# giuliojiang/pbrt-v3-IILE

Measured on AMD Instinct MI355X. Metric: Mray/s on killeroo-simple 1080p (path integrator, rays = Scene::Intersect + IntersectP calls), higher is better.
Workload: dtype f32

## Files before the change

pbrt-v3-iile_amd/csrc/device/dbsdf.h:

```cpp
#pragma once
enum Lobe : int { kLobePassThrough, kLobeLambert, kLobeLambertTrans, kLobeMicro, kLobeMicroTrans, kLobeBlend, kLobeSpecular, kLobeSpecTrans };
DEV bool lobe_is_specular(Lobe l) { return l == kLobePassThrough || l == kLobeSpecular || l == kLobeSpecTrans; }
struct Bsdf {
    F3 ns, ng, ss, ts;
    F3 kd;
    union { F3 micro_r, ks; };
    union { F3 kr, ltrans_t, cond_eta; };
    union { F3 kt, mtrans_t, cond_k; };
    float alpha, eta;
    float alpha_y;
    F3 t0;
    bool has_t0, has_t1;
    float path_eta;
    bool has_mtrans;
    int n_lobes;
    float on_a, on_b;
    bool oren_nayar;
    int mtype;
    bool has_lambert, has_micro, has_spec;
    bool has_blend;
    bool has_ltrans;
};
DEV int n_nonspec(const Bsdf &b) {
    return (b.has_lambert ? 1 : 0) + (b.has_ltrans ? 1 : 0) + (b.has_micro ? 1 : 0) + (b.has_mtrans ? 1 : 0) + (b.has_blend ? 1 : 0);
// ... 214 lines not shown
    *slope_y = Sg * z * sqrtf(1.f + *slope_x * *slope_x);
}
DEV F3 tr_sample_wh(F3 wo, float u0, float u1, float ax, float ay) {
    bool flip = wo.z < 0;
    F3 wi = flip ? -wo : wo;
    F3 ws = normalize(F3{ax * wi.x, ay * wi.y, wi.z});
    float sx, sy;
    tr_sample11(ws.z, u0, u1, &sx, &sy);
    float tmp = cos_phi(ws) * sx - sin_phi(ws) * sy;
    sy = sin_phi(ws) * sx + cos_phi(ws) * sy;
    sx = tmp;
    sx = ax * sx;
    sy = ay * sy;
    F3 wh = normalize(F3{-sx, -sy, 1.f});
    if (flip) wh = -wh;
    return wh;
}
DEV F3 micro_f(const Bsdf &b, F3 wo, F3 wi) {
    float cos_o = fabsf(wo.z), cos_i = fabsf(wi.z);
    F3 wh = wi + wo;
    if (cos_i == 0 || cos_o == 0) return F3{0, 0, 0};
    if (wh.x == 0 && wh.y == 0 && wh.z == 0) return F3{0, 0, 0};
    wh = normalize(wh);
    F3 F;
    if (b.mtype == kMatMetal) {
        F = fr_conductor(fabsf(dot(wi, wh)), b.cond_eta, b.cond_k);
    } else {
        float Fr = (b.mtype == kMatUber || b.mtype == kMatGlass || b.mtype == kMatTranslucent) ? fr_dielectric(dot(wi, wh), 1.f, b.eta)
                                                                                              : fr_dielectric(dot(wi, wh), 1.5f, 1.f);
        F = F3{Fr, Fr, Fr};
    }
    return sdiv(b.micro_r * tr_d(wh, b.alpha, b.alpha_y) * tr_g(wo, wi, b.alpha, b.alpha_y) * F, 4 * cos_i * cos_o);
}
DEV float micro_pdf(const Bsdf &b, F3 wo, F3 wi) {
    if (!same_hemisphere(wo, wi)) return 0;
    F3 wh = normalize(wo + wi);
    return tr_pdf(wo, wh, b.alpha, b.alpha_y) / (4 * dot(wo, wh));
}
DEV float pow5(float v) { return (v * v) * (v * v) * v; }
DEV F3 blend_f(const Bsdf &b, F3 wo, F3 wi) {
    const F3 one = F3{1.f, 1.f, 1.f};
    const F3 diffuse = (28.f / (23.f * kPi)) * b.kd * (one - b.ks) * (1 - pow5(1 - .5f * fabsf(wi.z))) * (1 - pow5(1 - .5f * fabsf(wo.z)));
    F3 wh = wi + wo;
    if (wh.x == 0 && wh.y == 0 && wh.z == 0) return F3{0, 0, 0};
    wh = normalize(wh);
    const float s = tr_d(wh, b.alpha, b.alpha_y) / (4 * absdot(wi, wh) * mx(fabsf(wi.z), fabsf(wo.z)));
    const F3 schlick = b.ks + pow5(1 - dot(wi, wh)) * (one - b.ks);
    return diffuse + s * schlick;
}
DEV float blend_pdf(const Bsdf &b, F3 wo, F3 wi) {
    if (!same_hemisphere(wo, wi)) return 0;
    const F3 wh = normalize(wo + wi);
    const float pdf_wh = tr_pdf(wo, wh, b.alpha, b.alpha_y);
    return .5f * (fabsf(wi.z) * kInvPi + pdf_wh / (4 * dot(wo, wh)));
}
DEV F3 diffuse_f(const Bsdf &b, F3 wo, F3 wi) {
    if (!b.oren_nayar) return b.kd * kInvPi;
    const float sin_i = sin_theta(wi), sin_o = sin_theta(wo);
    float max_cos = 0;
    if (double(sin_i) > 1e-4 && double(sin_o) > 1e-4) {
        const float sin_phi_i = sin_phi(wi), cos_phi_i = cos_phi(wi);
        const float sin_phi_o = sin_phi(wo), cos_phi_o = cos_phi(wo);
        const float d_cos = cos_phi_i * cos_phi_o + sin_phi_i * sin_phi_o;
        max_cos = mx(0.f, d_cos);
    }
    float sin_alpha, tan_beta;
    if (fabsf(wi.z) > fabsf(wo.z)) {
        sin_alpha = sin_o;
        tan_beta = sin_i / fabsf(wi.z);
    } else {
        sin_alpha = sin_i;
        tan_beta = sin_o / fabsf(wo.z);
    }
    return b.kd * kInvPi * (b.on_a + b.on_b * max_cos * sin_alpha * tan_beta);
}
DEV float lambert_pdf(F3 wo, F3 wi) { return same_hemisphere(wo, wi) ? fabsf(wi.z) * kInvPi : 0; }
DEV F3 ltrans_f(const Bsdf &b) { return b.ltrans_t * kInvPi; }
DEV float ltrans_pdf(F3 wo, F3 wi) { return !same_hemisphere(wo, wi) ? fabsf(wi.z) * kInvPi : 0; }
DEV bool refract_dir(F3 wi, F3 n, float eta, F3 *wt) {
    const float cos_i = dot(n, wi);
    const float sin2_i = mx(0.f, 1 - cos_i * cos_i);
    const float sin2_t = eta * eta * sin2_i;
    if (sin2_t >= 1) return false;
    const float cos_t = sqrtf(1 - sin2_t);
    *wt = eta * -wi + (eta * cos_i - cos_t) * n;
    return true;
}
DEV bool specular_refract(F3 wo, float eta_a, float eta_b, F3 *wi, float *scale) {
    const bool entering = wo.z > 0;
    const float eta_i = entering ? eta_a : eta_b, eta_t = entering ? eta_b : eta_a;
    const F3 n = (wo.z < 0.f) ? -F3{0, 0, 1} : F3{0, 0, 1};
    if (!refract_dir(wo, n, eta_i / eta_t, wi)) return false;
    *scale = (eta_i * eta_i) / (eta_t * eta_t);
    return true;
}
DEV F3 mtrans_f(const Bsdf &b, F3 wo, F3 wi) {
    if (same_hemisphere(wo, wi)) return F3{0, 0, 0};
    const float cos_o = wo.z, cos_i = wi.z;
    if (cos_i == 0 || cos_o == 0) return F3{0, 0, 0};
    const float eta_a = 1.f, eta_b = b.eta;
    const float eta = wo.z > 0 ? (eta_b / eta_a) : (eta_a / eta_b);
    F3 wh = normalize(wo + wi * eta);
    if (wh.z < 0) wh = -wh;
    const float F = fr_dielectric(dot(wo, wh), eta_a, eta_b);
    const float sqrt_denom = dot(wo, wh) + eta * dot(wi, wh);
    const float factor = 1 / eta;
    const float omf = 1.f - F;
    return F3{omf, omf, omf} * b.mtrans_t *
           fabsf(tr_d(wh, b.alpha, b.alpha_y) * tr_g(wo, wi, b.alpha, b.alpha_y) * eta * eta * absdot(wi, wh) * absdot(wo, wh) * factor * factor /
                 (cos_i * cos_o * sqrt_denom * sqrt_denom));
}
DEV float mtrans_pdf(const Bsdf &b, F3 wo, F3 wi) {
    if (same_hemisphere(wo, wi)) return 0;
    const float eta_a = 1.f, eta_b = b.eta;
    const float eta = wo.z > 0 ? (eta_b / eta_a) : (eta_a / eta_b);
    const F3 wh = normalize(wo + wi * eta);
    const float sqrt_denom = dot(wo, wh) + eta * dot(wi, wh);
    const float dwh_dwi = fabsf((eta * eta * dot(wi, wh)) / (sqrt_denom * sqrt_denom));
    return tr_pdf(wo, wh, b.alpha, b.alpha_y) * dwh_dwi;
}
DEV F3 lobes_f(const Bsdf &b, F3 wo, F3 wi) {
    F3 f = F3{0, 0, 0};
    if (b.has_lambert) f = f + diffuse_f(b, wo, wi);
    if (b.has_micro) f = f + micro_f(b, wo, wi);
    if (b.has_blend) f = f + blend_f(b, wo, wi);
    return f;
}
DEV F3 trans_lobes_f(const Bsdf &b, F3 wo, F3 wi) {
    F3 f = F3{0, 0, 0};
    if (b.has_ltrans) f = f + ltrans_f(b);
    if (b.has_mtrans) f = f + mtrans_f(b, wo, wi);
    return f;
}
DEV F3 bsdf_f(const Bsdf &b, F3 woW, F3 wiW) {
    F3 wi = to_local(b, wiW), wo = to_local(b, woW);
    if (wo.z == 0) return F3{0, 0, 0};
    bool reflect = dot(wiW, b.ng) * dot(woW, b.ng) > 0;
    if (reflect) return lobes_f(b, wo, wi);
    return trans_lobes_f(b, wo, wi);
}
DEV float bsdf_pdf(const Bsdf &b, F3 woW, F3 wiW) {
    if (b.n_lobes == 0) return 0.f;
    F3 wo = to_local(b, woW), wi = to_local(b, wiW);
    if (wo.z == 0) return 0.f;
    float pdf = 0.f;
    if (b.has_lambert) pdf += lambert_pdf(wo, wi);
    if (b.has_ltrans) pdf += ltrans_pdf(wo, wi);
    if (b.has_micro) pdf += micro_pdf(b, wo, wi);
    if (b.has_mtrans) pdf += mtrans_pdf(b, wo, wi);
    if (b.has_blend) pdf += blend_pdf(b, wo, wi);
    const int matching = n_nonspec(b);
    return matching > 0 ? pdf / matching : 0.f;
}
DEV F3 bsdf_sample_f(const Bsdf &b, F3 woW, F3 *wiW, float u0, float u1, float *pdf, const bool allow_specular = false,
                     bool *sampled_specular = nullptr, bool *sampled_transmission = nullptr) {
    if (sampled_specular) *sampled_specular = false;
    if (sampled_transmission) *sampled_transmission = false;
    const int matching = allow_specular ? b.n_lobes : n_nonspec(b);
    if (matching == 0) {
        *pdf = 0;
        return F3{0, 0, 0};
    }
    int comp = int(floorf(u0 * matching));
    if (comp > matching - 1) comp = matching - 1;
    Lobe pick;
    int count = comp;
    if (allow_specular && b.has_t0 && count-- == 0)
        pick = kLobePassThrough;
    else if (b.has_lambert && count-- == 0)
        pick = kLobeLambert;
    else if (b.has_ltrans && count-- == 0)
        pick = kLobeLambertTrans;
    else if (b.has_micro && count-- == 0)
        pick = kLobeMicro;
    else if (b.has_mtrans && count-- == 0)
        pick = kLobeMicroTrans;
    else if (b.has_blend && count-- == 0)
        pick = kLobeBlend;
    else if (!(allow_specular && b.has_t1) || (b.has_spec && count-- == 0))
        pick = kLobeSpecular;
    else
        pick = kLobeSpecTrans;
    if (pick == kLobeSpecular && !b.has_spec) __builtin_unreachable();
    const float ur0 = mn(u0 * matching - comp, kOneMinusEpsilon);
    F3 wo = to_local(b, woW);
    if (wo.z == 0) return F3{0, 0, 0};
    *pdf = 0;
    F3 wi = F3{0, 0, 0}, f;
    if (pick == kLobeLambert) {
        wi = cosine_sample_hemisphere(ur0, u1);
        if (wo.z < 0) wi.z *= -1;
        *pdf = lambert_pdf(wo, wi);
        f = diffuse_f(b, wo, wi);
    } else if (pick == kLobeLambertTrans) {
        wi = cosine_sample_hemisphere(ur0, u1);
        if (wo.z > 0) wi.z *= -1;
        *pdf = ltrans_pdf(wo, wi);
        f = ltrans_f(b);
    } else if (pick == kLobeMicro) {
        F3 wh = tr_sample_wh(wo, ur0, u1, b.alpha, b.alpha_y);
        wi = -wo + 2 * dot(wo, wh) * wh;
        if (!same_hemisphere(wo, wi))
            f = F3{0, 0, 0};
        else {
            *pdf = tr_pdf(wo, wh, b.alpha, b.alpha_y) / (4 * dot(wo, wh));
            f = micro_f(b, wo, wi);
        }
    } else if (pick == kLobeBlend) {
        float ua = ur0;
        if (ua < .5f) {
            ua = mn(2 * ua, kOneMinusEpsilon);
            wi = cosine_sample_hemisphere(ua, u1);
            if (wo.z < 0) wi.z *= -1;
        } else {
            ua = mn(2 * (ua - .5f), kOneMinusEpsilon);
            const F3 wh = tr_sample_wh(wo, ua, u1, b.alpha, b.alpha_y);
            wi = -wo + 2 * dot(wo, wh) * wh;
            if (!same_hemisphere(wo, wi)) return F3{0, 0, 0};
        }
        *pdf = blend_pdf(b, wo, wi);
        f = blend_f(b, wo, wi);
    } else if (pick == kLobeMicroTrans) {
        const F3 wh = tr_sample_wh(wo, ur0, u1, b.alpha, b.alpha_y);
        const float eta_a = 1.f, eta_b = b.eta;
        const float eta = wo.z > 0 ? (eta_a / eta_b) : (eta_b / eta_a);
        if (!refract_dir(wo, wh, eta, &wi)) return F3{0, 0, 0};
        *pdf = mtrans_pdf(b, wo, wi);
        f = mtrans_f(b, wo, wi);
    } else if (pick == kLobePassThrough || pick == kLobeSpecTrans) {
        const float eta_a = 1.f, eta_b = pick == kLobePassThrough ? 1.f : b.eta;
        float scale;
        if (!specular_refract(wo, eta_a, eta_b, &wi, &scale)) return F3{0, 0, 0};
        *pdf = 1;
        const F3 ft = (pick == kLobePassThrough ? b.t0 : b.kt) * (1.f - fr_dielectric(wi.z, eta_a, eta_b));
        f = sdiv(ft * scale, fabsf(wi.z));
        if (sampled_specular) *sampled_specular = true;
        if (sampled_transmission) *sampled_transmission = true;
    } else if (b.mtype == kMatGlass) {
        const float eta_a = 1.f, eta_b = b.eta;
        const float F = fr_dielectric(wo.z, eta_a, eta_b);
        if (ur0 < F) {
            wi = F3{-wo.x, -wo.y, wo.z};
            *pdf = F;
            f = sdiv(F * b.kr, fabsf(wi.z));
        } else {
            float scale;
            if (!specular_refract(wo, eta_a, eta_b, &wi, &scale)) return F3{0, 0, 0};
            const F3 ft = b.kt * (1 - F);
            *pdf = 1 - F;
            f = sdiv(ft * scale, fabsf(wi.z));
            if (sampled_transmission) *sampled_transmission = true;
        }
        if (sampled_specular) *sampled_specular = true;
    } else {
        wi = F3{-wo.x, -wo.y, wo.z};
        *pdf = 1;
        const float fr = b.mtype == kMatMirror ? 1.f : fr_dielectric(wi.z, 1.f, b.eta);
        f = sdiv(F3{fr, fr, fr} * b.kr, fabsf(wi.z));
        if (sampled_specular) *sampled_specular = true;
    }
    if (*pdf == 0) {
        if (sampled_specular) *sampled_specular = false;
        if (sampled_transmission) *sampled_transmission = false;
        return F3{0, 0, 0};
    }
    *wiW = to_world(b, wi);
    const bool glossy = !lobe_is_specular(pick);
    if (glossy && matching > 1) {
        if (pick != kLobeLambert && b.has_lambert) *pdf += lambert_pdf(wo, wi);
        if (pick != kLobeLambertTrans && b.has_ltrans) *pdf += ltrans_pdf(wo, wi);
        if (pick != kLobeMicro && b.has_micro) *pdf += micro_pdf(b, wo, wi);
        if (pick != kLobeMicroTrans && b.has_mtrans) *pdf += mtrans_pdf(b, wo, wi);
    }
    if (matching > 1) *pdf /= matching;
    if (glossy && matching > 1) {
        bool reflect = dot(*wiW, b.ng) * dot(woW, b.ng) > 0;
        f = reflect ? lobes_f(b, wo, wi) : trans_lobes_f(b, wo, wi);
    }
    return f;
}

enum DisneyLobe : int { kDzDiffuse, kDzFakeSS, kDzRetro, kDzSheen, kDzMicro, kDzCoat, kDzMicroTrans, kDzLambertTrans };
struct DisneyBsdf : Bsdf {
    bool disney;
    bool dz_diffuse;
    bool dz_thin, dz_sheen, dz_coat;
    bool dz_trans_smith;
    F3 r_diffuse, r_ss, r_retro, r_sheen;
    F3 cspec0;
    float metallic, rough;
    float coat_w, coat_alpha;
    float t_ax, t_ay;
};
template <bool DIS>
struct bsdf_of { using type = Bsdf; };
template <>
struct bsdf_of<true> { using type = DisneyBsdf; };
DEV float lerpf(float t, float a, float b) { return (1 - t) * a + t * b; }
DEV F3 lerp3(float t, F3 a, F3 b) { return (1 - t) * a + t * b; }
DEV float sqr(float x) { return x * x; }
DEV float schlick_weight(float cos_theta) {
    const float m = clampf(1 - cos_theta, 0, 1);
    return (m * m) * (m * m) * m;
}
DEV float fr_schlick(float r0, float cos_theta) { return lerpf(schlick_weight(cos_theta), r0, 1.f); }
DEV F3 fr_schlick3(F3 r0, float cos_theta) { return lerp3(schlick_weight(cos_theta), r0, F3{1.f, 1.f, 1.f}); }
DEV float schlick_r0_from_eta(float eta) { return sqr(eta - 1) / sqr(eta + 1); }

DEV void make_disney(const DMaterial &m, const iile_disney &dz, DisneyBsdf *b) {
    b->disney = true;
    b->mtype = kMatDisney;
    b->t0 = b->kd = F3{0, 0, 0};
    b->has_t0 = b->has_t1 = b->has_lambert = b->has_spec = b->has_blend = b->oren_nayar = false;
    b->on_a = 1.f, b->on_b = 0.f;
    b->path_eta = 1.f;
    const F3 c = clamp0(m.kd);
    const float metallic_w = dz.metallic;
    const float e = m.eta;
    const float strans = dz.spec_trans;
    const float diffuse_w = (1 - metallic_w) * (1 - strans);
    const float dt = dz.diff_trans / 2;
    const float rough = m.alpha;
    const float lum = lum_y(c);
    const F3 one = F3{1.f, 1.f, 1.f};
    const F3 ctint = lum > 0 ? sdiv(c, lum) : one;
    const float sheen_w = dz.sheen;
    F3 csheen = F3{0, 0, 0};
    if (sheen_w > 0) csheen = lerp3(dz.sheen_tint, one, ctint);
    int n = 0;
    b->dz_thin = dz.thin != 0;
    b->dz_diffuse = diffuse_w > 0;
    b->dz_sheen = false;
    b->r_diffuse = b->r_ss = b->r_retro = b->r_sheen = F3{0, 0, 0};
    b->rough = rough;
    if (b->dz_diffuse) {
        if (b->dz_thin) {
            const float flat = dz.flatness;
            b->r_diffuse = (diffuse_w * (1 - flat) * (1 - dt)) * c;
            b->r_ss = (diffuse_w * flat * (1 - dt)) * c;
            n += 2;
        } else {
            b->r_diffuse = diffuse_w * c;
            ++n;
        }
        b->r_retro = diffuse_w * c;
        ++n;
        if (sheen_w > 0) {
            b->dz_sheen = true;
            b->r_sheen = (diffuse_w * sheen_w) * csheen;
            ++n;
        }
    }
    const float aspect = float(sqrt(1. - double(dz.anisotropic) * .9));
    b->alpha = mx(.001f, sqr(rough) / aspect);
    b->alpha_y = mx(.001f, sqr(rough) * aspect);
    b->cspec0 = lerp3(metallic_w, schlick_r0_from_eta(e) * lerp3(dz.specular_tint, one, ctint), c);
    b->metallic = metallic_w;
    b->eta = e;
    b->micro_r = c;
    b->has_micro = true;
    ++n;
    b->dz_coat = dz.clearcoat > 0;
    b->coat_w = dz.clearcoat;
    b->coat_alpha = lerpf(dz.clearcoat_gloss, .1f, .001f);
    if (b->dz_coat) ++n;
    b->has_mtrans = strans > 0;
    b->mtrans_t = F3{0, 0, 0};
    b->t_ax = b->alpha, b->t_ay = b->alpha_y;
    b->dz_trans_smith = false;
    if (b->has_mtrans) {
        b->mtrans_t = strans * F3{sqrtf(c.x), sqrtf(c.y), sqrtf(c.z)};
        if (b->dz_thin) {
            const float rscaled = (0.65f * e - 0.35f) * rough;
            b->t_ax = mx(.001f, sqr(rscaled) / aspect);
            b->t_ay = mx(.001f, sqr(rscaled) * aspect);
            b->dz_trans_smith = true;
        }
        ++n;
    }
    b->has_ltrans = b->dz_thin;
    b->ltrans_t = F3{0, 0, 0};
    if (b->dz_thin) {
        b->ltrans_t = dt * c;
        ++n;
    }
    b->n_lobes = n;
}
template <bool EXT, bool DIS>
DEV typename bsdf_of<DIS>::type make_bsdf_at(const DScene &S, int material, const DMaterial &m, const Isect &is) {
    if constexpr (!DIS) {
        return make_bsdf<EXT>(m, is);
    } else {
        DisneyBsdf b;
        if (m.type == kMatDisney) {
            b.ns = is.sn;
            b.ng = is.n;
            b.ss = normalize(is.sdpdu);
            b.ts = cross(b.ns, b.ss);
            make_disney(m, disney_table(S)[material], &b);
        } else {
            static_cast<Bsdf &>(b) = make_bsdf<EXT>(m, is);
            b.disney = false;
        }
        return b;
    }
}
DEV int n_nonspec(const DisneyBsdf &b) { return b.disney ? b.n_lobes : n_nonspec(static_cast<const Bsdf &>(b)); }
DEV F3 dz_diffuse_f(F3 R, F3 wo, F3 wi) {
    const float Fo = schlick_weight(fabsf(wo.z)), Fi = schlick_weight(fabsf(wi.z));
    return R * kInvPi * (1 - Fo / 2) * (1 - Fi / 2);
}
DEV F3 dz_fakess_f(F3 R, float roughness, F3 wo, F3 wi) {
    F3 wh = wi + wo;
    if (wh.x == 0 && wh.y == 0 && wh.z == 0) return F3{0, 0, 0};
    wh = normalize(wh);
    const float cos_d = dot(wi, wh);
    const float Fss90 = cos_d * cos_d * roughness;
    const float Fo = schlick_weight(fabsf(wo.z)), Fi = schlick_weight(fabsf(wi.z));
    const float Fss = lerpf(Fo, 1.f, Fss90) * lerpf(Fi, 1.f, Fss90);
    const float ss = 1.25f * (Fss * (1 / (fabsf(wo.z) + fabsf(wi.z)) - .5f) + .5f);
    return R * kInvPi * ss;
}
DEV F3 dz_retro_f(F3 R, float roughness, F3 wo, F3 wi) {
    F3 wh = wi + wo;
    if (wh.x == 0 && wh.y == 0 && wh.z == 0) return F3{0, 0, 0};
    wh = normalize(wh);
    const float cos_d = dot(wi, wh);
    const float Fo = schlick_weight(fabsf(wo.z)), Fi = schlick_weight(fabsf(wi.z));
    const float Rr = 2 * roughness * cos_d * cos_d;
    return R * kInvPi * Rr * (Fo + Fi + Fo * Fi * (Rr - 1));
}
DEV F3 dz_sheen_f(F3 R, F3 wo, F3 wi) {
    F3 wh = wi + wo;
    if (wh.x == 0 && wh.y == 0 && wh.z == 0) return F3{0, 0, 0};
    wh = normalize(wh);
    return R * schlick_weight(dot(wi, wh));
}
DEV float gtr1(float cos_theta, float alpha) {
    const float alpha2 = alpha * alpha;
    return (alpha2 - 1) / (kPi * log_f(alpha2) * (1 + (alpha2 - 1) * cos_theta * cos_theta));
}
DEV float smith_g_ggx(float cos_theta, float alpha) {
    const float alpha2 = alpha * alpha;
    const float cos2 = cos_theta * cos_theta;
    return 1 / (cos_theta + sqrtf(alpha2 + cos2 - alpha2 * cos2));
}
DEV F3 dz_coat_f(const DisneyBsdf &b, F3 wo, F3 wi) {
    F3 wh = wi + wo;
    if (wh.x == 0 && wh.y == 0 && wh.z == 0) return F3{0, 0, 0};
    wh = normalize(wh);
    const float Dr = gtr1(fabsf(wh.z), b.coat_alpha);
    const float Fr = fr_schlick(.04f, dot(wo, wh));
    const float Gr = smith_g_ggx(fabsf(wo.z), .25f) * smith_g_ggx(fabsf(wi.z), .25f);
    const float v = float(.25 * double(b.coat_w) * double(Gr) * double(Fr) * double(Dr));
    return F3{v, v, v};
}
DEV float dz_coat_pdf(const DisneyBsdf &b, F3 wo, F3 wi) {
    if (!same_hemisphere(wo, wi)) return 0;
    F3 wh = wi + wo;
    if (wh.x == 0 && wh.y == 0 && wh.z == 0) return 0;
    wh = normalize(wh);
    const float Dr = gtr1(fabsf(wh.z), b.coat_alpha);
    return Dr / (4 * dot(wo, wh));
}
DEV F3 dz_micro_f(const DisneyBsdf &b, F3 wo, F3 wi) {
    const float cos_o = fabsf(wo.z), cos_i = fabsf(wi.z);
    F3 wh = wi + wo;
    if (cos_i == 0 || cos_o == 0) return F3{0, 0, 0};
    if (wh.x == 0 && wh.y == 0 && wh.z == 0) return F3{0, 0, 0};
    wh = normalize(wh);
    const float cos_h = dot(wi, wh);
    const float fd = fr_dielectric(cos_h, 1.f, b.eta);
    const F3 F = lerp3(b.metallic, F3{fd, fd, fd}, fr_schlick3(b.cspec0, cos_h));
    const float G = tr_g1(wo, b.alpha, b.alpha_y) * tr_g1(wi, b.alpha, b.alpha_y);
    return sdiv(b.micro_r * tr_d(wh, b.alpha, b.alpha_y) * G * F, 4 * cos_i * cos_o);
}
DEV F3 dz_mtrans_f(const DisneyBsdf &b, F3 wo, F3 wi) {
    if (same_hemisphere(wo, wi)) return F3{0, 0, 0};
    const float cos_o = wo.z, cos_i = wi.z;
    if (cos_i == 0 || cos_o == 0) return F3{0, 0, 0};
    const float eta_a = 1.f, eta_b = b.eta;
    const float eta = wo.z > 0 ? (eta_b / eta_a) : (eta_a / eta_b);
    F3 wh = normalize(wo + wi * eta);
    if (wh.z < 0) wh = -wh;
    const float F = fr_dielectric(dot(wo, wh), eta_a, eta_b);
    const float sqrt_denom = dot(wo, wh) + eta * dot(wi, wh);
    const float factor = 1 / eta;
    const float omf = 1.f - F;
    const float G = b.dz_trans_smith ? tr_g(wo, wi, b.t_ax, b.t_ay) : tr_g1(wo, b.t_ax, b.t_ay) * tr_g1(wi, b.t_ax, b.t_ay);
    return F3{omf, omf, omf} * b.mtrans_t *
           fabsf(tr_d(wh, b.t_ax, b.t_ay) * G * eta * eta * absdot(wi, wh) * absdot(wo, wh) * factor * factor /
                 (cos_i * cos_o * sqrt_denom * sqrt_denom));
}
DEV float dz_mtrans_pdf(const DisneyBsdf &b, F3 wo, F3 wi) {
    if (same_hemisphere(wo, wi)) return 0;
    const float eta_a = 1.f, eta_b = b.eta;
    const float eta = wo.z > 0 ? (eta_b / eta_a) : (eta_a / eta_b);
    const F3 wh = normalize(wo + wi * eta);
    const float sqrt_denom = dot(wo, wh) + eta * dot(wi, wh);
    const float dwh_dwi = fabsf((eta * eta * dot(wi, wh)) / (sqrt_denom * sqrt_denom));
    return tr_pdf(wo, wh, b.t_ax, b.t_ay) * dwh_dwi;
}
DEV F3 dz_lobe_f(const DisneyBsdf &b, DisneyLobe l, F3 wo, F3 wi) {
    switch (l) {
    case kDzDiffuse: return dz_diffuse_f(b.r_diffuse, wo, wi);
    case kDzFakeSS: return dz_fakess_f(b.r_ss, b.rough, wo, wi);
    case kDzRetro: return dz_retro_f(b.r_retro, b.rough, wo, wi);
    case kDzSheen: return dz_sheen_f(b.r_sheen, wo, wi);
    case kDzMicro: return dz_micro_f(b, wo, wi);
    case kDzCoat: return dz_coat_f(b, wo, wi);
    case kDzMicroTrans: return dz_mtrans_f(b, wo, wi);
    default: return ltrans_f(b);
    }
}
DEV bool dz_has(const DisneyBsdf &b, DisneyLobe l) {
    switch (l) {
    case kDzDiffuse:
    case kDzRetro: return b.dz_diffuse;
    case kDzFakeSS: return b.dz_diffuse && b.dz_thin;
    case kDzSheen: return b.dz_sheen;
    case kDzMicro: return true;
    case kDzCoat: return b.dz_coat;
    case kDzMicroTrans: return b.has_mtrans;
    default: return b.has_ltrans;
    }
}
DEV F3 dz_lobes_f(const DisneyBsdf &b, bool reflect, F3 wo, F3 wi) {
    F3 f = F3{0, 0, 0};
    if (reflect) {
        if (b.dz_diffuse) {
            f = f + dz_diffuse_f(b.r_diffuse, wo, wi);
            if (b.dz_thin) f = f + dz_fakess_f(b.r_ss, b.rough, wo, wi);
            f = f + dz_retro_f(b.r_retro, b.rough, wo, wi);
            if (b.dz_sheen) f = f + dz_sheen_f(b.r_sheen, wo, wi);
        }
        f = f + dz_micro_f(b, wo, wi);
        if (b.dz_coat) f = f + dz_coat_f(b, wo, wi);
    } else {
        if (b.has_mtrans) f = f + dz_mtrans_f(b, wo, wi);
        if (b.has_ltrans) f = f + ltrans_f(b);
    }
    return f;
}
DEV float dz_lobes_pdf(const DisneyBsdf &b, int skip, F3 wo, F3 wi, float pdf) {
    const float cosine = lambert_pdf(wo, wi);
#pragma unroll
    for (int l = kDzDiffuse; l <= kDzSheen; ++l)
        if (l != skip && dz_has(b, DisneyLobe(l))) pdf += cosine;
    if (skip != kDzMicro) pdf += micro_pdf(b, wo, wi);
    if (skip != kDzCoat && b.dz_coat) pdf += dz_coat_pdf(b, wo, wi);
    if (skip != kDzMicroTrans && b.has_mtrans) pdf += dz_mtrans_pdf(b, wo, wi);
    if (skip != kDzLambertTrans && b.has_ltrans) pdf += ltrans_pdf(wo, wi);
    return pdf;
}
DEV F3 bsdf_f(const DisneyBsdf &b, F3 woW, F3 wiW) {
    if (!b.disney) return bsdf_f(static_cast<const Bsdf &>(b), woW, wiW);
    const F3 wi = to_local(b, wiW), wo = to_local(b, woW);
    if (wo.z == 0) return F3{0, 0, 0};
    const bool reflect = dot(wiW, b.ng) * dot(woW, b.ng) > 0;
    return dz_lobes_f(b, reflect, wo, wi);
}
DEV float bsdf_pdf(const DisneyBsdf &b, F3 woW, F3 wiW) {
    if (!b.disney) return bsdf_pdf(static_cast<const Bsdf &>(b), woW, wiW);
    const F3 wo = to_local(b, woW), wi = to_local(b, wiW);
    if (wo.z == 0) return 0.f;
    return dz_lobes_pdf(b, -1, wo, wi, 0.f) / b.n_lobes;
}
DEV F3 bsdf_sample_f(const DisneyBsdf &b, F3 woW, F3 *wiW, float u0, float u1, float *pdf, const bool allow_specular = false,
                     bool *sampled_specular = nullptr, bool *sampled_transmission = nullptr) {
    if (!b.disney) return bsdf_sample_f(static_cast<const Bsdf &>(b), woW, wiW, u0, u1, pdf, allow_specular, sampled_specular, sampled_transmission);
    if (sampled_specular) *sampled_specular = false;
    if (sampled_transmission) *sampled_transmission = false;
    const int matching = b.n_lobes;
    int comp = int(floorf(u0 * matching));
    if (comp > matching - 1) comp = matching - 1;
    int pick = kDzLambertTrans, count = comp;
    bool found = false;
#pragma unroll
    for (int l = kDzDiffuse; l <= kDzLambertTrans; ++l)
        if (!found && dz_has(b, DisneyLobe(l)) && count-- == 0) pick = l, found = true;
    const float ur0 = mn(u0 * matching - comp, kOneMinusEpsilon);
    const F3 wo = to_local(b, woW);
    if (wo.z == 0) return F3{0, 0, 0};
    *pdf = 0;
    F3 wi = F3{0, 0, 0}, f;
    if (pick <= kDzSheen) {
        wi = cosine_sample_hemisphere(ur0, u1);
        if (wo.z < 0) wi.z *= -1;
        *pdf = lambert_pdf(wo, wi);
        f = dz_lobe_f(b, DisneyLobe(pick), wo, wi);
    } else if (pick == kDzMicro) {
        const F3 wh = tr_sample_wh(wo, ur0, u1, b.alpha, b.alpha_y);
        wi = -wo + 2 * dot(wo, wh) * wh;
        if (!same_hemisphere(wo, wi))
            f = F3{0, 0, 0};
        else {
            *pdf = tr_pdf(wo, wh, b.alpha, b.alpha_y) / (4 * dot(wo, wh));
            f = dz_micro_f(b, wo, wi);
        }
    } else if (pick == kDzCoat) {
        const float alpha2 = .25f * .25f;
        const float cos_t = sqrtf(mx(0.f, (1 - powf(alpha2, 1 - ur0)) / (1 - alpha2)));
        const float sin_t = sqrtf(mx(0.f, 1 - cos_t * cos_t));
        const float phi = 2 * kPi * u1;
        float sp, cp;
        sincos_f(phi, &sp, &cp);
        F3 wh = F3{sin_t * cp, sin_t * sp, cos_t};
        if (!same_hemisphere(wo, wh)) wh = -wh;
        wi = -wo + 2 * dot(wo, wh) * wh;
        if (!same_hemisphere(wo, wi))
            f = F3{0, 0, 0};
        else {
            *pdf = dz_coat_pdf(b, wo, wi);
            f = dz_coat_f(b, wo, wi);
        }
    } else if (pick == kDzMicroTrans) {
        const F3 wh = tr_sample_wh(wo, ur0, u1, b.t_ax, b.t_ay);
        const float eta_a = 1.f, eta_b = b.eta;
        const float eta = wo.z > 0 ? (eta_a / eta_b) : (eta_b / eta_a);
        if (!refract_dir(wo, wh, eta, &wi)) return F3{0, 0, 0};
        *pdf = dz_mtrans_pdf(b, wo, wi);
        f = dz_mtrans_f(b, wo, wi);
    } else {
        wi = cosine_sample_hemisphere(ur0, u1);
        if (wo.z > 0) wi.z *= -1;
        *pdf = ltrans_pdf(wo, wi);
        f = ltrans_f(b);
    }
    if (*pdf == 0) return F3{0, 0, 0};
    *wiW = to_world(b, wi);
    if (matching > 1) {
        *pdf = dz_lobes_pdf(b, pick, wo, wi, *pdf);
        *pdf /= matching;
        const bool reflect = dot(*wiW, b.ng) * dot(woW, b.ng) > 0;
        f = dz_lobes_f(b, reflect, wo, wi);
    }
    if (sampled_transmission) *sampled_transmission = false;
    return f;
}
```

pbrt-v3-iile_amd/csrc/device/dpath.h:

```cpp
#pragma once
#include "dscene.h"

namespace iile {

DEV uint32_t div_magic(uint32_t a, uint32_t magic, uint32_t shift) {
    uint32_t t = __umulhi(magic, a);
    return (t + ((a - t) >> 1)) >> shift;
}

DEV uint32_t halton_index(const DScene &S, int px, int py, uint32_t k) {
    int pmx = px - (px / 128) * 128, pmy = py - (py / 128) * 128;
    if (pmx < 0) pmx += 128;
    if (pmy < 0) pmy += 128;
    return S.pixel_offsets[pmy * 128 + pmx] + k * uint32_t(S.sample_stride);
}

DEV float radical_inverse_base2(uint32_t a) {
    unsigned long long rev = (unsigned long long)__brev(a) << 32;
    return float(double(rev) * 0x1p-64);
}
DEV float radical_inverse_base3(uint32_t a0) {
    const float inv_base = 1.f / 3.f;
    double a = double(a0), reversed = 0;
    float inv_base_n = 1;
// ... 740 lines not shown
        const DSphere &sp = S.spheres[shape];
        sphere_test(sp, ro, rd, IILE_INF, &t, &od, &ph);
        sphere_interaction<DIFFS>(sp, od, ph, is);
    }
}

DEV void triangle_interaction(const DScene &S, int prim, uint32_t flags, F3 p0, F3 p1, F3 p2, F3 ray_d, float b0,
                              float b1, float b2, Isect *is) {
    float uv00 = 0, uv01 = 0, uv10 = 1, uv11 = 0, uv20 = 1, uv21 = 1;
    if (flags & 4u) {
        const float2 *u = S.tri_uv + 3 * size_t(prim);
        float2 a = u[0], b = u[1], c = u[2];
        uv00 = a.x;
        uv01 = a.y;
        uv10 = b.x;
        uv11 = b.y;
        uv20 = c.x;
        uv21 = c.y;
    }
    float duv02x = uv00 - uv20, duv02y = uv01 - uv21;
    float duv12x = uv10 - uv20, duv12y = uv11 - uv21;
    F3 dp02 = p0 - p2, dp12 = p1 - p2;
    float determinant = duv02x * duv12y - duv02y * duv12x;
    bool degenerate = double(fabsf(determinant)) < 1e-8;
    F3 dpdu = F3{0, 0, 0}, dpdv = F3{0, 0, 0};
    if (!degenerate) {
        float invdet = 1 / determinant;
        dpdu = (duv12y * dp02 - duv02y * dp12) * invdet;
        dpdv = (-duv12x * dp02 + duv02x * dp12) * invdet;
    }
    if (degenerate || length_sq(cross(dpdu, dpdv)) == 0)
        coordinate_system(normalize(cross(p2 - p0, p1 - p0)), &dpdu, &dpdv);
    float xs = (fabsf(b0 * p0.x) + fabsf(b1 * p1.x) + fabsf(b2 * p2.x));
    float ys = (fabsf(b0 * p0.y) + fabsf(b1 * p1.y) + fabsf(b2 * p2.y));
    float zs = (fabsf(b0 * p0.z) + fabsf(b1 * p1.z) + fabsf(b2 * p2.z));
    is->perr = kGamma7 * F3{xs, ys, zs};
    is->p = b0 * p0 + b1 * p1 + b2 * p2;
    is->u = b0 * uv00 + b1 * uv10 + b2 * uv20;
    is->v = b0 * uv01 + b1 * uv11 + b2 * uv21;
    is->dpdu = dpdu;
    is->dpdv = dpdv;
    is->wo = normalize(-ray_d);
    F3 n = normalize(cross(dp02, dp12));
    const bool flip = (flags & 8u) != 0;
    if (flags & 2u) {
        const float4 *nn = S.tri_norms + 3 * size_t(prim);
        float4 a = nn[0], b = nn[1], c = nn[2];
        F3 n0 = F3{a.x, a.y, a.z}, n1 = F3{b.x, b.y, b.z}, n2 = F3{c.x, c.y, c.z};
        F3 ns = (b0 * n0 + b1 * n1 + b2 * n2);
        if (length_sq(ns) > 0)
            ns = normalize(ns);
        else
            ns = n;
        F3 ss = normalize(dpdu);
        F3 ts = cross(ss, ns);
        if (length_sq(ts) > 0.f) {
            ts = normalize(ts);
            ss = cross(ts, ns);
        } else
            coordinate_system(ns, &ss, &ts);
        const F3 dn1 = n0 - n2, dn2 = n1 - n2;
        if (double(fabsf(determinant)) < 1e-8) {
            is->dndu = is->dndv = F3{0, 0, 0};
        } else {
            const float inv_det = 1 / determinant;
            is->dndu = (duv12y * dn1 - duv02y * dn2) * inv_det;
            is->dndv = (-duv12x * dn1 + duv02x * dn2) * inv_det;
        }
        F3 sn = normalize(cross(ss, ts));
        if (flip) sn = -sn;
        n = faceforward(n, sn);
        is->sn = sn;
        is->sdpdu = ss;
        is->sdpdv = ts;
    } else {
        if (flip) n = -n;
        is->sn = n;
        is->sdpdu = dpdu;
        is->sdpdv = dpdv;
        is->dndu = is->dndv = F3{0, 0, 0};
    }
    is->flip = flip;
    is->n = n;
}

#include "dtrav.h"
#include "dtex.h"
#include "dbsdf.h"
#include "dlight.h"

template <bool EXT, bool COUNT, class BSDF>
DEV uint32_t estimate_direct_request(const DScene &S, const DLight &lt, const DSphere *lsp, const Isect &is, const BSDF &bsdf, float ul0,
                                     float ul1, float us0, float us1, F3 &so, F3 &sd, F3 &A, F3 &mo, F3 &md, F3 &Bc,
                                     unsigned long long *n_pdf_tests, unsigned long long *n_pdf_hits) {
    uint32_t nee_flags = 0;
    if (EXT && lt.type == kLightInfinite) {
        float light_pdf = 0, scattering_pdf = 0;
        F3 wi = F3{0, 0, 0}, target = F3{0, 0, 0};
        const F3 Li = inf_sample_li(S, lt, is.p, ul0, ul1, &wi, &light_pdf, &target);
        if (light_pdf > 0 && !is_black(Li)) {
            const F3 f = bsdf_f(bsdf, is.wo, wi) * absdot(wi, is.sn);
            scattering_pdf = bsdf_pdf(bsdf, is.wo, wi);
            if (!is_black(f)) {
                so = offset_ray_origin(is.p, is.perr, is.n, target - is.p);
                sd = target - so;
                A = sdiv(f * Li * power_heuristic(light_pdf, scattering_pdf), light_pdf);
                nee_flags |= NEE_HAS_SHADOW;
            }
        }
        F3 f2 = bsdf_sample_f(bsdf, is.wo, &wi, us0, us1, &scattering_pdf);
        f2 = f2 * absdot(wi, is.sn);
        if (!is_black(f2) && scattering_pdf > 0) {
            const float lp = inf_pdf_li(S, lt, wi);
            if (lp != 0) {
                mo = offset_ray_origin(is.p, is.perr, is.n, wi);
                md = wi;
                Bc = sdiv(f2 * inf_le(S, lt, wi) * power_heuristic(scattering_pdf, lp), scattering_pdf);
                nee_flags |= NEE_HAS_MIS;
            }
        }
    } else if (EXT && iile_light_is_delta(lt.type)) {
        F3 wi, target;
        const F3 Li = delta_light_li(S, lt, is.p, &wi, &target);
        if (!is_black(Li)) {
            const F3 f = bsdf_f(bsdf, is.wo, wi) * absdot(wi, is.sn);
            if (!is_black(f)) {
                so = offset_ray_origin(is.p, is.perr, is.n, target - is.p);
                sd = target - so;
                A = sdiv(f * Li, 1.f);
                nee_flags |= NEE_HAS_SHADOW;
            }
        }
    } else {
        float light_pdf = 0, scattering_pdf = 0;
        F3 wi = F3{0, 0, 0}, Li = F3{0, 0, 0};
        const LightSample ps = EXT ? shape_sample(S, lt, is, ul0, ul1, &light_pdf) : sphere_sample(*lsp, is, ul0, ul1, &light_pdf);
        if (light_pdf == 0 || length_sq(ps.p - is.p) == 0) {
            light_pdf = 0;
        } else {
            wi = normalize(ps.p - is.p);
            Li = area_light_L(lt, ps.n, -wi);
        }
        if (light_pdf > 0 && !is_black(Li)) {
            const F3 f = bsdf_f(bsdf, is.wo, wi) * absdot(wi, is.sn);
            scattering_pdf = bsdf_pdf(bsdf, is.wo, wi);
            if (!is_black(f)) {
                so = offset_ray_origin(is.p, is.perr, is.n, ps.p - is.p);
                const F3 target = offset_ray_origin(ps.p, ps.perr, ps.n, so - ps.p);
                sd = target - so;
                A = sdiv(f * Li * power_heuristic(light_pdf, scattering_pdf), light_pdf);
                nee_flags |= NEE_HAS_SHADOW;
            }
        }
        F3 f2 = bsdf_sample_f(bsdf, is.wo, &wi, us0, us1, &scattering_pdf);
        f2 = f2 * absdot(wi, is.sn);
        if (!is_black(f2) && scattering_pdf > 0) {
            const F3 m_o = offset_ray_origin(is.p, is.perr, is.n, wi);
            bool can_reach = true;
            if (!COUNT && lt.type == kLightDiffuseArea) {
                float t_l;
                F3 od_l, ph_l;
                can_reach = sphere_test(lsp ? *lsp : S.spheres[lt.sphere], m_o, wi, IILE_INF, &t_l, &od_l, &ph_l);
            } else if (EXT && !COUNT && lt.type == kLightAreaQuadric) {
                float t_l;
                F3 od_l, ph_l;
                can_reach = quadric_test(S.quadrics[lt.quadric], m_o, wi, IILE_INF, &t_l, &od_l, &ph_l);
            }
            if (can_reach) {
                const float lp = EXT ? shape_pdf(S, lt, is, wi, n_pdf_tests, n_pdf_hits) : sphere_pdf(*lsp, is, wi);
                if (lp != 0) {
                    mo = m_o;
                    md = wi;
                    Bc = sdiv(f2 * F3{lt.lemit[0], lt.lemit[1], lt.lemit[2]} * power_heuristic(scattering_pdf, lp), scattering_pdf);
                    nee_flags |= NEE_HAS_MIS;
                }
            }
        }
    }
    return nee_flags;
}

DEV bool mis_ray_lit(const DScene &S, int li, int prim, float b0, float b1, float b2, F3 mo, F3 md) {
    const DLight &lt = S.lights[li];
    Isect lis;
    if (lt.type == kLightAreaTriangle) {
        const float4 v0 = S.tri_verts[3 * size_t(prim)], v1 = S.tri_verts[3 * size_t(prim) + 1], v2 = S.tri_verts[3 * size_t(prim) + 2];
        triangle_interaction(S, prim, f2b(v0.w), F3{v0.x, v0.y, v0.z}, F3{v1.x, v1.y, v1.z}, F3{v2.x, v2.y, v2.z}, md, b0, b1, b2, &lis);
    } else {
        shape_hit_interaction(S, lt.type == kLightAreaQuadric ? ~lt.quadric : lt.sphere, mo, md, &lis);
    }
    return lt.two_sided || dot(lis.n, -md) > 0;
}

}
```

Measured before the change: 12030.

## Split BSDF sampling into direction and evaluation to skip eval for unreachable MIS rays

Splits bsdf_sample_f into bsdf_sample_dir (choose lobe and direction) and bsdf_sample_eval (pdf and f). In light sampling, the MIS path now tests whether the sampled direction can reach the light, and for triangle lights computes the light pdf, before running the BSDF evaluation, so f/pdf work is skipped for directions that miss the light. Adds a struct carried between the two phases, which can raise register pressure and add divergence.

```diff
diff --git a/pbrt-v3-iile_amd/csrc/device/dbsdf.h b/pbrt-v3-iile_amd/csrc/device/dbsdf.h
--- a/pbrt-v3-iile_amd/csrc/device/dbsdf.h
+++ b/pbrt-v3-iile_amd/csrc/device/dbsdf.h
@@ -390,15 +390,19 @@
     const int matching = n_nonspec(b);
     return matching > 0 ? pdf / matching : 0.f;
 }
-DEV F3 bsdf_sample_f(const Bsdf &b, F3 woW, F3 *wiW, float u0, float u1, float *pdf, const bool allow_specular = false,
-                     bool *sampled_specular = nullptr, bool *sampled_transmission = nullptr) {
-    if (sampled_specular) *sampled_specular = false;
-    if (sampled_transmission) *sampled_transmission = false;
+struct BsdfDir {
+    int matching;
+    int pick;
+    F3 wi;
+    F3 wh;
+    float fr;
+    float scale;
+    bool refracted;
+};
+enum : int { kDirKeepPdf = -1, kDirNone = 0, kDirOk = 1 };
+DEV int bsdf_sample_dir(const Bsdf &b, F3 woW, float u0, float u1, const bool allow_specular, BsdfDir *d, F3 *wiW) {
     const int matching = allow_specular ? b.n_lobes : n_nonspec(b);
-    if (matching == 0) {
-        *pdf = 0;
-        return F3{0, 0, 0};
-    }
+    if (matching == 0) return kDirNone;
     int comp = int(floorf(u0 * matching));
     if (comp > matching - 1) comp = matching - 1;
     Lobe pick;
@@ -422,28 +426,21 @@
     if (pick == kLobeSpecular && !b.has_spec) __builtin_unreachable();
     const float ur0 = mn(u0 * matching - comp, kOneMinusEpsilon);
     F3 wo = to_local(b, woW);
-    if (wo.z == 0) return F3{0, 0, 0};
-    *pdf = 0;
-    F3 wi = F3{0, 0, 0}, f;
+    if (wo.z == 0) return kDirKeepPdf;
+    F3 wi = F3{0, 0, 0};
+    d->wh = F3{0, 0, 0};
+    d->fr = d->scale = 0;
+    d->refracted = false;
     if (pick == kLobeLambert) {
         wi = cosine_sample_hemisphere(ur0, u1);
         if (wo.z < 0) wi.z *= -1;
-        *pdf = lambert_pdf(wo, wi);
-        f = diffuse_f(b, wo, wi);
     } else if (pick == kLobeLambertTrans) {
         wi = cosine_sample_hemisphere(ur0, u1);
         if (wo.z > 0) wi.z *= -1;
-        *pdf = ltrans_pdf(wo, wi);
-        f = ltrans_f(b);
     } else if (pick == kLobeMicro) {
-        F3 wh = tr_sample_wh(wo, ur0, u1, b.alpha, b.alpha_y);
-        wi = -wo + 2 * dot(wo, wh) * wh;
-        if (!same_hemisphere(wo, wi))
-            f = F3{0, 0, 0};
-        else {
-            *pdf = tr_pdf(wo, wh, b.alpha, b.alpha_y) / (4 * dot(wo, wh));
-            f = micro_f(b, wo, wi);
-        }
+        d->wh = tr_sample_wh(wo, ur0, u1, b.alpha, b.alpha_y);
+        wi = -wo + 2 * dot(wo, d->wh) * d->wh;
+        if (!same_hemisphere(wo, wi)) return kDirNone;
     } else if (pick == kLobeBlend) {
         float ua = ur0;
         if (ua < .5f) {
@@ -454,47 +451,61 @@
             ua = mn(2 * (ua - .5f), kOneMinusEpsilon);
             const F3 wh = tr_sample_wh(wo, ua, u1, b.alpha, b.alpha_y);
             wi = -wo + 2 * dot(wo, wh) * wh;
-            if (!same_hemisphere(wo, wi)) return F3{0, 0, 0};
+            if (!same_hemisphere(wo, wi)) return kDirNone;
         }
-        *pdf = blend_pdf(b, wo, wi);
-        f = blend_f(b, wo, wi);
     } else if (pick == kLobeMicroTrans) {
         const F3 wh = tr_sample_wh(wo, ur0, u1, b.alpha, b.alpha_y);
         const float eta_a = 1.f, eta_b = b.eta;
         const float eta = wo.z > 0 ? (eta_a / eta_b) : (eta_b / eta_a);
-        if (!refract_dir(wo, wh, eta, &wi)) return F3{0, 0, 0};
-        *pdf = mtrans_pdf(b, wo, wi);
-        f = mtrans_f(b, wo, wi);
+        if (!refract_dir(wo, wh, eta, &wi)) return kDirNone;
     } else if (pick == kLobePassThrough || pick == kLobeSpecTrans) {
         const float eta_a = 1.f, eta_b = pick == kLobePassThrough ? 1.f : b.eta;
-        float scale;
-        if (!specular_refract(wo, eta_a, eta_b, &wi, &scale)) return F3{0, 0, 0};
+        if (!specular_refract(wo, eta_a, eta_b, &wi, &d->scale)) return kDirNone;
+    } else if (b.mtype == kMatGlass) {
+        const float eta_a = 1.f, eta_b = b.eta;
+        d->fr = fr_dielectric(wo.z, eta_a, eta_b);
+        if (ur0 < d->fr) {
+            wi = F3{-wo.x, -wo.y, wo.z};
+        } else {
+            if (!specular_refract(wo, eta_a, eta_b, &wi, &d->scale)) return kDirNone;
+            d->refracted = true;
+        }
+    } else {
+        wi = F3{-wo.x, -wo.y, wo.z};
+    }
+    d->matching = matching;
+    d->pick = pick;
+    d->wi = wi;
+    *wiW = to_world(b, wi);
+    return kDirOk;
+}
+DEV F3 bsdf_sample_eval(const Bsdf &b, F3 woW, F3 wiW, const BsdfDir &d, float *pdf, bool *sampled_specular = nullptr,
+                        bool *sampled_transmission = nullptr, F3 *wi_out = nullptr) {
+    const int matching = d.matching;
+    const Lobe pick = Lobe(d.pick);
+    if (pick == kLobeSpecular && !b.has_spec) __builtin_unreachable();
+    const F3 wo = to_local(b, woW), wi = d.wi;
+    const bool glossy = !lobe_is_specular(pick);
+    if (pick == kLobeLambert) {
+        *pdf = lambert_pdf(wo, wi);
+    } else if (pick == kLobeLambertTrans) {
+        *pdf = ltrans_pdf(wo, wi);
+    } else if (pick == kLobeMicro) {
+        *pdf = tr_pdf(wo, d.wh, b.alpha, b.alpha_y) / (4 * dot(wo, d.wh));
+    } else if (pick == kLobeBlend) {
+        *pdf = blend_pdf(b, wo, wi);
+    } else if (pick == kLobeMicroTrans) {
+        *pdf = mtrans_pdf(b, wo, wi);
+    } else if (pick == kLobePassThrough || pick == kLobeSpecTrans) {
         *pdf = 1;
-        const F3 ft = (pick == kLobePassThrough ? b.t0 : b.kt) * (1.f - fr_dielectric(wi.z, eta_a, eta_b));
-        f = sdiv(ft * scale, fabsf(wi.z));
         if (sampled_specular) *sampled_specular = true;
         if (sampled_transmission) *sampled_transmission = true;
     } else if (b.mtype == kMatGlass) {
-        const float eta_a = 1.f, eta_b = b.eta;
-        const float F = fr_dielectric(wo.z, eta_a, eta_b);
-        if (ur0 < F) {
-            wi = F3{-wo.x, -wo.y, wo.z};
-            *pdf = F;
-            f = sdiv(F * b.kr, fabsf(wi.z));
-        } else {
-            float scale;
-            if (!specular_refract(wo, eta_a, eta_b, &wi, &scale)) return F3{0, 0, 0};
-            const F3 ft = b.kt * (1 - F);
-            *pdf = 1 - F;
-            f = sdiv(ft * scale, fabsf(wi.z));
-            if (sampled_transmission) *sampled_transmission = true;
-        }
+        *pdf = d.refracted ? 1 - d.fr : d.fr;
+        if (sampled_transmission && d.refracted) *sampled_transmission = true;
         if (sampled_specular) *sampled_specular = true;
     } else {
-        wi = F3{-wo.x, -wo.y, wo.z};
         *pdf = 1;
-        const float fr = b.mtype == kMatMirror ? 1.f : fr_dielectric(wi.z, 1.f, b.eta);
-        f = sdiv(F3{fr, fr, fr} * b.kr, fabsf(wi.z));
         if (sampled_specular) *sampled_specular = true;
     }
     if (*pdf == 0) {
@@ -502,8 +513,7 @@
         if (sampled_transmission) *sampled_transmission = false;
         return F3{0, 0, 0};
     }
-    *wiW = to_world(b, wi);
-    const bool glossy = !lobe_is_specular(pick);
+    if (wi_out) *wi_out = wiW;
     if (glossy && matching > 1) {
         if (pick != kLobeLambert && b.has_lambert) *pdf += lambert_pdf(wo, wi);
         if (pick != kLobeLambertTrans && b.has_ltrans) *pdf += ltrans_pdf(wo, wi);
@@ -512,10 +522,40 @@
     }
     if (matching > 1) *pdf /= matching;
     if (glossy && matching > 1) {
-        bool reflect = dot(*wiW, b.ng) * dot(woW, b.ng) > 0;
-        f = reflect ? lobes_f(b, wo, wi) : trans_lobes_f(b, wo, wi);
-    }
-    return f;
+        bool reflect = dot(wiW, b.ng) * dot(woW, b.ng) > 0;
+        return reflect ? lobes_f(b, wo, wi) : trans_lobes_f(b, wo, wi);
+    }
+    if (pick == kLobeLambert) return diffuse_f(b, wo, wi);
+    if (pick == kLobeLambertTrans) return ltrans_f(b);
+    if (pick == kLobeMicro) return micro_f(b, wo, wi);
+    if (pick == kLobeBlend) return blend_f(b, wo, wi);
+    if (pick == kLobeMicroTrans) return mtrans_f(b, wo, wi);
+    if (pick == kLobePassThrough || pick == kLobeSpecTrans) {
+        const float eta_a = 1.f, eta_b = pick == kLobePassThrough ? 1.f : b.eta;
+        const F3 ft = (pick == kLobePassThrough ? b.t0 : b.kt) * (1.f - fr_dielectric(wi.z, eta_a, eta_b));
+        return sdiv(ft * d.scale, fabsf(wi.z));
+    }
+    if (b.mtype == kMatGlass) {
+        const float F = d.fr;
+        if (!d.refracted) return sdiv(F * b.kr, fabsf(wi.z));
+        const F3 ft = b.kt * (1 - F);
+        return sdiv(ft * d.scale, fabsf(wi.z));
+    }
+    const float fr = b.mtype == kMatMirror ? 1.f : fr_dielectric(wi.z, 1.f, b.eta);
+    return sdiv(F3{fr, fr, fr} * b.kr, fabsf(wi.z));
+}
+DEV F3 bsdf_sample_f(const Bsdf &b, F3 woW, F3 *wiW, float u0, float u1, float *pdf, const bool allow_specular = false,
+                     bool *sampled_specular = nullptr, bool *sampled_transmission = nullptr) {
+    if (sampled_specular) *sampled_specular = false;
+    if (sampled_transmission) *sampled_transmission = false;
+    BsdfDir d;
+    F3 w;
+    const int have = bsdf_sample_dir(b, woW, u0, u1, allow_specular, &d, &w);
+    if (have != kDirOk) {
+        if (have == kDirNone) *pdf = 0;
+        return F3{0, 0, 0};
+    }
+    return bsdf_sample_eval(b, woW, w, d, pdf, sampled_specular, sampled_transmission, wiW);
 }
 
 enum DisneyLobe : int { kDzDiffuse, kDzFakeSS, kDzRetro, kDzSheen, kDzMicro, kDzCoat, kDzMicroTrans, kDzLambertTrans };
@@ -804,11 +844,8 @@
     if (wo.z == 0) return 0.f;
     return dz_lobes_pdf(b, -1, wo, wi, 0.f) / b.n_lobes;
 }
-DEV F3 bsdf_sample_f(const DisneyBsdf &b, F3 woW, F3 *wiW, float u0, float u1, float *pdf, const bool allow_specular = false,
-                     bool *sampled_specular = nullptr, bool *sampled_transmission = nullptr) {
-    if (!b.disney) return bsdf_sample_f(static_cast<const Bsdf &>(b), woW, wiW, u0, u1, pdf, allow_specular, sampled_specular, sampled_transmission);
-    if (sampled_specular) *sampled_specular = false;
-    if (sampled_transmission) *sampled_transmission = false;
+DEV int bsdf_sample_dir(const DisneyBsdf &b, F3 woW, float u0, float u1, const bool allow_specular, BsdfDir *d, F3 *wiW) {
+    if (!b.disney) return bsdf_sample_dir(static_cast<const Bsdf &>(b), woW, u0, u1, allow_specular, d, wiW);
     const int matching = b.n_lobes;
     int comp = int(floorf(u0 * matching));
     if (comp > matching - 1) comp = matching - 1;
@@ -819,23 +856,18 @@
         if (!found && dz_has(b, DisneyLobe(l)) && count-- == 0) pick = l, found = true;
     const float ur0 = mn(u0 * matching - comp, kOneMinusEpsilon);
     const F3 wo = to_local(b, woW);
-    if (wo.z == 0) return F3{0, 0, 0};
-    *pdf = 0;
-    F3 wi = F3{0, 0, 0}, f;
+    if (wo.z == 0) return kDirKeepPdf;
+    F3 wi = F3{0, 0, 0};
+    d->wh = F3{0, 0, 0};
+    d->fr = d->scale = 0;
+    d->refracted = false;
     if (pick <= kDzSheen) {
         wi = cosine_sample_hemisphere(ur0, u1);
         if (wo.z < 0) wi.z *= -1;
-        *pdf = lambert_pdf(wo, wi);
-        f = dz_lobe_f(b, DisneyLobe(pick), wo, wi);
     } else if (pick == kDzMicro) {
-        const F3 wh = tr_sample_wh(wo, ur0, u1, b.alpha, b.alpha_y);
-        wi = -wo + 2 * dot(wo, wh) * wh;
-        if (!same_hemisphere(wo, wi))
-            f = F3{0, 0, 0};
-        else {
-            *pdf = tr_pdf(wo, wh, b.alpha, b.alpha_y) / (4 * dot(wo, wh));
-            f = dz_micro_f(b, wo, wi);
-        }
+        d->wh = tr_sample_wh(wo, ur0, u1, b.alpha, b.alpha_y);
+        wi = -wo + 2 * dot(wo, d->wh) * d->wh;
+        if (!same_hemisphere(wo, wi)) return kDirNone;
     } else if (pick == kDzCoat) {
         const float alpha2 = .25f * .25f;
         const float cos_t = sqrtf(mx(0.f, (1 - powf(alpha2, 1 - ur0)) / (1 - alpha2)));
@@ -846,33 +878,62 @@
         F3 wh = F3{sin_t * cp, sin_t * sp, cos_t};
         if (!same_hemisphere(wo, wh)) wh = -wh;
         wi = -wo + 2 * dot(wo, wh) * wh;
-        if (!same_hemisphere(wo, wi))
-            f = F3{0, 0, 0};
-        else {
-            *pdf = dz_coat_pdf(b, wo, wi);
-            f = dz_coat_f(b, wo, wi);
-        }
+        if (!same_hemisphere(wo, wi)) return kDirNone;
     } else if (pick == kDzMicroTrans) {
         const F3 wh = tr_sample_wh(wo, ur0, u1, b.t_ax, b.t_ay);
         const float eta_a = 1.f, eta_b = b.eta;
         const float eta = wo.z > 0 ? (eta_a / eta_b) : (eta_b / eta_a);
-        if (!refract_dir(wo, wh, eta, &wi)) return F3{0, 0, 0};
-        *pdf = dz_mtrans_pdf(b, wo, wi);
-        f = dz_mtrans_f(b, wo, wi);
+        if (!refract_dir(wo, wh, eta, &wi)) return kDirNone;
     } else {
         wi = cosine_sample_hemisphere(ur0, u1);
         if (wo.z > 0) wi.z *= -1;
+    }
+    d->matching = matching;
+    d->pick = pick;
+    d->wi = wi;
+    *wiW = to_world(b, wi);
+    return kDirOk;
+}
+DEV F3 bsdf_sample_eval(const DisneyBsdf &b, F3 woW, F3 wiW, const BsdfDir &d, float *pdf, bool *sampled_specular = nullptr,
+                        bool *sampled_transmission = nullptr, F3 *wi_out = nullptr) {
+    if (!b.disney) return bsdf_sample_eval(static_cast<const Bsdf &>(b), woW, wiW, d, pdf, sampled_specular, sampled_transmission, wi_out);
+    const int matching = d.matching, pick = d.pick;
+    const F3 wo = to_local(b, woW), wi = d.wi;
+    if (pick <= kDzSheen)
+        *pdf = lambert_pdf(wo, wi);
+    else if (pick == kDzMicro)
+        *pdf = tr_pdf(wo, d.wh, b.alpha, b.alpha_y) / (4 * dot(wo, d.wh));
+    else if (pick == kDzCoat)
+        *pdf = dz_coat_pdf(b, wo, wi);
+    else if (pick == kDzMicroTrans)
+        *pdf = dz_mtrans_pdf(b, wo, wi);
+    else
         *pdf = ltrans_pdf(wo, wi);
-        f = ltrans_f(b);
-    }
     if (*pdf == 0) return F3{0, 0, 0};
-    *wiW = to_world(b, wi);
+    if (wi_out) *wi_out = wiW;
     if (matching > 1) {
         *pdf = dz_lobes_pdf(b, pick, wo, wi, *pdf);
         *pdf /= matching;
-        const bool reflect = dot(*wiW, b.ng) * dot(woW, b.ng) > 0;
-        f = dz_lobes_f(b, reflect, wo, wi);
-    }
+        const bool reflect = dot(wiW, b.ng) * dot(woW, b.ng) > 0;
+        return dz_lobes_f(b, reflect, wo, wi);
+    }
+    if (pick <= kDzSheen) return dz_lobe_f(b, DisneyLobe(pick), wo, wi);
+    if (pick == kDzMicro) return dz_micro_f(b, wo, wi);
+    if (pick == kDzCoat) return dz_coat_f(b, wo, wi);
+    if (pick == kDzMicroTrans) return dz_mtrans_f(b, wo, wi);
+    return ltrans_f(b);
+}
+DEV F3 bsdf_sample_f(const DisneyBsdf &b, F3 woW, F3 *wiW, float u0, float u1, float *pdf, const bool allow_specular = false,
+                     bool *sampled_specular = nullptr, bool *sampled_transmission = nullptr) {
+    if (!b.disney) return bsdf_sample_f(static_cast<const Bsdf &>(b), woW, wiW, u0, u1, pdf, allow_specular, sampled_specular, sampled_transmission);
+    if (sampled_specular) *sampled_specular = false;
     if (sampled_transmission) *sampled_transmission = false;
-    return f;
-}
+    BsdfDir d;
+    F3 w;
+    const int have = bsdf_sample_dir(b, woW, u0, u1, allow_specular, &d, &w);
+    if (have != kDirOk) {
+        if (have == kDirNone) *pdf = 0;
+        return F3{0, 0, 0};
+    }
+    return bsdf_sample_eval(b, woW, w, d, pdf, nullptr, nullptr, wiW);
+}
diff --git a/pbrt-v3-iile_amd/csrc/device/dpath.h b/pbrt-v3-iile_amd/csrc/device/dpath.h
--- a/pbrt-v3-iile_amd/csrc/device/dpath.h
+++ b/pbrt-v3-iile_amd/csrc/device/dpath.h
@@ -916,27 +916,49 @@
                 nee_flags |= NEE_HAS_SHADOW;
             }
         }
-        F3 f2 = bsdf_sample_f(bsdf, is.wo, &wi, us0, us1, &scattering_pdf);
-        f2 = f2 * absdot(wi, is.sn);
-        if (!is_black(f2) && scattering_pdf > 0) {
-            const F3 m_o = offset_ray_origin(is.p, is.perr, is.n, wi);
-            bool can_reach = true;
-            if (!COUNT && lt.type == kLightDiffuseArea) {
-                float t_l;
-                F3 od_l, ph_l;
-                can_reach = sphere_test(lsp ? *lsp : S.spheres[lt.sphere], m_o, wi, IILE_INF, &t_l, &od_l, &ph_l);
-            } else if (EXT && !COUNT && lt.type == kLightAreaQuadric) {
-                float t_l;
-                F3 od_l, ph_l;
-                can_reach = quadric_test(S.quadrics[lt.quadric], m_o, wi, IILE_INF, &t_l, &od_l, &ph_l);
-            }
-            if (can_reach) {
+        if (COUNT) {
+            F3 f2 = bsdf_sample_f(bsdf, is.wo, &wi, us0, us1, &scattering_pdf);
+            f2 = f2 * absdot(wi, is.sn);
+            if (!is_black(f2) && scattering_pdf > 0) {
                 const float lp = EXT ? shape_pdf(S, lt, is, wi, n_pdf_tests, n_pdf_hits) : sphere_pdf(*lsp, is, wi);
                 if (lp != 0) {
-                    mo = m_o;
+                    mo = offset_ray_origin(is.p, is.perr, is.n, wi);
                     md = wi;
                     Bc = sdiv(f2 * F3{lt.lemit[0], lt.lemit[1], lt.lemit[2]} * power_heuristic(scattering_pdf, lp), scattering_pdf);
                     nee_flags |= NEE_HAS_MIS;
+                }
+            }
+        } else {
+            BsdfDir dir;
+            if (bsdf_sample_dir(bsdf, is.wo, us0, us1, false, &dir, &wi) == kDirOk) {
+                const F3 m_o = offset_ray_origin(is.p, is.perr, is.n, wi);
+                bool can_reach = true;
+                float lp = 0;
+                const bool tri = EXT && lt.type != kLightDiffuseArea && lt.type != kLightAreaQuadric;
+                if (lt.type == kLightDiffuseArea) {
+                    float t_l;
+                    F3 od_l, ph_l;
+                    can_reach = sphere_test(lsp ? *lsp : S.spheres[lt.sphere], m_o, wi, IILE_INF, &t_l, &od_l, &ph_l);
+                } else if (EXT && lt.type == kLightAreaQuadric) {
+                    float t_l;
+                    F3 od_l, ph_l;
+                    can_reach = quadric_test(S.quadrics[lt.quadric], m_o, wi, IILE_INF, &t_l, &od_l, &ph_l);
+                } else if (EXT) {
+                    lp = shape_pdf(S, lt, is, wi, n_pdf_tests, n_pdf_hits);
+                    can_reach = lp != 0;
+                }
+                if (can_reach) {
+                    F3 f2 = bsdf_sample_eval(bsdf, is.wo, wi, dir, &scattering_pdf);
+                    f2 = f2 * absdot(wi, is.sn);
+                    if (!is_black(f2) && scattering_pdf > 0) {
+                        if (!tri) lp = EXT ? shape_pdf(S, lt, is, wi, n_pdf_tests, n_pdf_hits) : sphere_pdf(*lsp, is, wi);
+                        if (lp != 0) {
+                            mo = m_o;
+                            md = wi;
+                            Bc = sdiv(f2 * F3{lt.lemit[0], lt.lemit[1], lt.lemit[2]} * power_heuristic(scattering_pdf, lp), scattering_pdf);
+                            nee_flags |= NEE_HAS_MIS;
+                        }
+                    }
                 }
             }
         }
```

After: 12060 (median of 6 runs). No clear change (+0.2%).
